# rvolden/C3POa

Measured on AMD Instinct MI355X. Metric: R2C2 reads->consensus/sec, higher is better.
Workload: dtype int32

## Files before the change

### c3poa_amd/csrc/c3_args.h

```cpp
#pragma once
#include "c3_dev.h"
#include <cstddef>

struct C3Counters {
  int queue;
  int peaks_queue;
  unsigned long long cells;
  unsigned long long cells_computed;
  unsigned long long zero_cells;
  int poa_ovf;
  int poa_ovf16;
  int n_windows;
  int win_ovf;
  int win_queue2;
  int band_layers, band_fallback;
  int band_mismatch;
  struct { int window, layer, R, q, band_row, full_row, next_row; } verify;
  unsigned long long phases[16];
};
static_assert(offsetof(C3Counters, cells) % 8 == 0 && offsetof(C3Counters, cells_computed) % 8 == 0 &&
              offsetof(C3Counters, zero_cells) % 8 == 0 && offsetof(C3Counters, phases) % 8 == 0, "u64 counters must be 8-byte aligned");

struct ConkArgs {
  C3Batch b; const uint8_t* sp_codes; const int* sp_len; int32_t* track; C3Info* info; C3Counters* cnt;
  int match, mismatch, penalty;
  int n_spl; int32_t* scan;
};
struct PeaksArgs {
  C3Batch b; const int32_t* track; C3Info* info; double* bufA; double* bufB; int32_t* cand; uint8_t* cstate;
  int32_t* raw_peaks; int32_t* n_raw; const int* sp_len; double coef[64]; int64_t maxL; int window, iters, min_dist;
  C3Counters* cnt;
};
struct PoaArgs {
  C3Batch b; C3Info* info; C3Params p; C3Counters* cnt; const int* work; int n_work;
  int* ibase; int* ebase; char* cellsb; uint8_t* bbase; long long* score;
  int Ncap, K, Pcap, cells_cap;
// ... 24 lines not shown
  C3Batch b; C3Info* info; C3Params p; C3Counters* cnt; const int* work; int n_work;
  const uint8_t* draft; int32_t* tpos; int wcap; uint8_t* eD; int64_t ecap; int* lw_first; int* lw_last; int NLcap, NWcap;
  WinRec* wrec; WLayer* wlay; int* win_base;
  int sub_shift;
  int rows_old;
};
struct WinArgs {
  C3Batch b; C3Params p; C3Counters* cnt; int n_win; const WinRec* wrec_in; WinRec* wrec; const WLayer* wlay; int NLcap;
  const uint8_t* draft;
  uint8_t* base; int* ibase; int* ebase; long long* score;
  int32_t* H; uint16_t* D; uint4* rdesc; int Ncap, K; long long hcap; uint8_t* wout; int wout_cap;
  int Lcap;
  int band_mode;
  const int* wlist; int* ovf_list;
  int no_chain;
};
#define W_INTS 19
struct WinLayout { size_t ints, edges, bases, score, H, D, desc, total; };
__host__ __device__ inline WinLayout c3_win_layout(size_t Ncap, size_t K, size_t hcap) {
  WinLayout l;
  l.ints = sizeof(int) * W_INTS * Ncap; l.edges = sizeof(int) * 4 * Ncap * K; l.bases = 2 * Ncap; l.score = sizeof(long long) * Ncap;
  l.H = sizeof(int32_t) * hcap; l.D = hcap; l.desc = sizeof(uint4) * (Ncap + 1);
  l.total = l.ints + l.edges + l.bases + l.score + l.H + l.D + l.desc;
  return l;
}
struct StitchArgs {
  C3Batch b; C3Info* info; const int* work; int n_work; const WinRec* wrec; const int* win_base; const uint8_t* wout; int wout_cap; char* cons;
  const uint8_t* zflag;
};
struct AdapterArgs {
// ... 33 lines not shown
```

### c3poa_amd/csrc/c3_handle.hip

```cpp
#include "c3_host.h"
#include "c3_bgzf.h"

thread_local double c3h::g_alloc_ms = 0.0;

__device__ __forceinline__ uint32_t pack_code(uint32_t b) {
  const uint32_t u = b & 0xDFu;
  const uint32_t c = (u >> 1) & 3u;
  const bool ok = (u == 'A') | (u == 'C') | (u == 'G') | (u == 'T') | (u == 'U');
  return ok ? (c ^ (c >> 1)) : 0u;
}
__global__ __launch_bounds__(256) void k_pack(const uint8_t* ascii, const int64_t* off, const int64_t* woff, int n, uint32_t* pk) {
  const int lane = threadIdx.x & 63;
  const int wave = (blockIdx.x * blockDim.x + threadIdx.x) >> 6, n_waves = (gridDim.x * blockDim.x) >> 6;
  for (int r = wave; r < n; r += n_waves) {
    const int64_t L = off[r + 1] - off[r];
    const int64_t nw = woff[r + 1] - woff[r];
    const uint8_t* s = ascii + off[r];
    uint32_t* dst = pk + woff[r];
    for (int64_t w = lane; w < nw; w += 64) {
      uint32_t x = 0;
      if (w * 16 + 16 <= L) {
        uint32_t v[4];
        __builtin_memcpy(v, s + w * 16, 16);
#pragma unroll
// ... 456 lines not shown
extern "C" int c3_debug_calibrate(c3_handle* h, long long bytes) {
  if (!h || bytes < 4096) return C3_E_ARG;
  HIPCHK(hipSetDevice(h->cfg.device));
  uint32_t *a = nullptr, *b = nullptr;
  HIPCHK(hipMalloc(&a, (size_t)bytes)); HIPCHK(hipMalloc(&b, (size_t)bytes));
  HIPCHK(hipMemsetAsync(a, 1, (size_t)bytes, h->stream));
  HIPCHK(hipStreamSynchronize(h->stream));
  hipLaunchKernelGGL(k_calib_rw, dim3(h->n_cus * 8), dim3(256), 0, h->stream, a, b, (size_t)bytes / 4);
  HIPCHK(hipStreamSynchronize(h->stream));
  HIPCHK(hipFree(a)); HIPCHK(hipFree(b));
  return C3_E_OK;
}

extern "C" int c3_debug_phases(c3_handle* h, int which, unsigned long long* out) {
  if (!h || !out) return C3_E_ARG;
  memcpy(out, which ? h->phase_win : h->phase_poa, 128);
  return C3_E_OK;
}

extern "C" int c3_batch_timing(c3_handle* h, c3_timing* t) { if (!h || !t) return C3_E_ARG; *t = h->tm; return C3_E_OK; }

extern "C" int c3_fetch_track(c3_handle* h, int read, int32_t* out, int64_t cap) {
  if (!h || read < 0 || read >= h->n || !out) return C3_E_ARG;
  if (!(h->stages_done & C3_STAGE_CONK)) return c3_fail(h, C3_E_STATE, "conk stage not run");
  int64_t L = h->off[read + 1] - h->off[read];
  if (cap < L) return C3_E_LIMIT;
  HIPCHK(hipSetDevice(h->cfg.device));
  HIPCHK(hipMemcpy(out, h->d_track.as<int32_t>() + h->off[read], sizeof(int32_t) * (size_t)L, hipMemcpyDeviceToHost));
  return (int)L;
}
extern "C" int c3_fetch_smoothed(c3_handle* h, int read, double* out, int64_t cap) {
// ... 60 lines not shown
```

### c3poa_amd/csrc/c3_host.h

```cpp
#pragma once
#include "c3_dev.h"
#include "c3_args.h"
#include "c3_launch.h"
#include "c3_checks.h"
#include "c3_emit.h"
#include "c3_post.h"
#include "c3_fastx.h"
#include "c3_dsplit.h"
#include "c3_bgzf.h"
#include <algorithm>
#include <atomic>
#include <chrono>
#include <cstddef>
#include <cstdio>
#include <cstdlib>
#include <cstring>
#include <functional>
#include <string>
#include <vector>

struct c3_handle;
namespace c3h {
extern thread_local double g_alloc_ms;
int qv_scratch(c3_handle* h, long long max_m, long long max_n, int n_items, QvArgs& a, int* grid);
// ... 119 lines not shown
  DBuf d_qv, s_qv_dirs, s_qv_g, d_qv_cnt, d_gather_qv;
  hipEvent_t ev_qv[2] = {nullptr, nullptr}; c3_qv_timing qtm = {}; bool snap_qv = false;
  DBuf d_post[16]; hipEvent_t ev_post[5] = {}; c3_post_timing ptm = {};
  PostText pt;
  DemuxText dx; std::vector<uint32_t> dmx_meta_host;
  DBuf d_fa[20]; hipEvent_t ev_fa[10] = {}; c3_demux_timing dtm = {}; struct C3FaHdr* h_fa_hdr = nullptr;
  DBuf d_emit[10]; c3h::EmitBufs emit_sa; c3_emit_timing etm = {};
  c3h::EmitBufs emit_snap; DBuf d_emit_names, d_emit_noff; c3h::ZStage emit_zs;
  hipEvent_t ev_emit_dn = nullptr;
  std::atomic<bool> emit_pending{false}; int emit_S = 0, emit_flags = 0; std::vector<int64_t> emit_so; c3_emit_timing emit_tm = {};
  std::vector<Summary> sum; std::vector<int> work;
  int res_prefix = 0;
  int peaks_grid = 0; bool debug_msa = false; bool injected = false;
  int n_windows = 0;
  c3_timing tm;
  unsigned long long phase_poa[16] = {0}, phase_win[16] = {0};
  int stages_done = 0;
};

static inline int c3_hip_fail(c3_handle* h, hipError_t e, const char* what, const char* file, int line) {
  char buf[512];
  const char* base = strrchr(file, '/');
  snprintf(buf, sizeof buf, "HIP error %d (%s) at %s:%d: %s", (int)e, hipGetErrorString(e), base ? base + 1 : file, line, what);
  if (h) h->err = buf;
  return C3_E_HIP;
}
static inline int c3_fail(c3_handle* h, int code, const char* msg) { if (h) h->err = msg; return code; }
#define HIPCHK(x) do { hipError_t e_ = (x); if (e_ != hipSuccess) return c3_hip_fail(h, e_, #x, __FILE__, __LINE__); } while (0)
static inline int host_fail(int code, const char* msg) { c3_set_host_error(msg); return code; }
static inline int bgzf_fail(hipError_t e, const char* what) {
  char buf[256];
// ... 57 lines not shown
```

### c3poa_amd/csrc/c3_stages.hip

```cpp
#include "c3_host.h"

__global__ void k_summary(const C3Info* info, const int64_t* off, int n, Summary* out) {
  int i = blockIdx.x * blockDim.x + threadIdx.x;
  if (i >= n) return;
  const C3Info* p = &info[i];
  Summary s; s.status = p->status; s.n_sub = p->n_sub; s.max_sub = 0; s.sum_sub = 0; s.max_dang = 0; s.n_peaks = p->n_peaks;
  for (int k = 0; k < p->n_sub; ++k) { int l = p->sub_end[k] - p->sub_beg[k]; s.sum_sub += l; if (l > s.max_sub) s.max_sub = l; }
  int L = (int)(off[i + 1] - off[i]);
  s.front = p->has_front ? p->front_end : 0; s.tail = p->has_tail ? L - p->tail_beg : 0;
  if (p->has_front) s.max_dang = p->front_end;
  if (p->has_tail && L - p->tail_beg > s.max_dang) s.max_dang = L - p->tail_beg;
  out[i] = s;
}

static hipError_t zero_counters(c3_handle* h) { return hipMemsetAsync(h->d_counter.p, 0, sizeof(C3Counters), h->stream); }

static int auto_slots(c3_handle* h, int want, size_t per_slot_bytes, int n_items, int waves_per_cu) {
  int s = want > 0 ? want : h->n_cus * waves_per_cu;
  size_t budget = h->mem_total ? h->mem_total / 3 : ((size_t)64 << 30);
  if (per_slot_bytes > 0) { size_t mx = budget / per_slot_bytes; if ((size_t)s > mx) s = (int)std::max<size_t>(mx, 1); }
  if (s > n_items) s = std::max(n_items, 1);
  return s;
}

// ... 304 lines not shown
      HIPCHK(h->s_win_h2.ensure(L2.H * S2)); HIPCHK(h->s_win_d2.ensure(L2.D * S2 + 256));
      HIPCHK(h->d_wovf.ensure(sizeof(int) * (size_t)n_win));
    }
    WinArgs a; memset(&a, 0, sizeof(a));
    a.b = dev_batch(h); a.p = dev_params(h->cfg); a.cnt = dev_cnt(h); a.n_win = n_win;
    a.wrec_in = h->d_wrec.as<WinRec>(); a.wrec = h->d_wrec.as<WinRec>(); a.wlay = h->d_wlay.as<WLayer>(); a.NLcap = NLcap;
    a.draft = h->d_draft.as<uint8_t>();
    a.ibase = h->s_win_i.as<int>(); a.ebase = h->s_win_nk.as<int>();
    a.base = h->s_win_b.as<uint8_t>(); a.score = h->s_win_sc.as<long long>();
    a.H = h->s_win_h.as<int32_t>(); a.D = h->s_win_d.as<uint16_t>(); a.rdesc = h->s_win_desc.as<uint4>(); a.Ncap = Ncap; a.K = K; a.hcap = hcap; a.Lcap = std::min(std::min(Ncap, 2 * WL + 30 * NLcap), ((getenv("C3_DEBUG_WIN_LDS") ? atoi(getenv("C3_DEBUG_WIN_LDS")) : 6656) - 16) / 6);
    if (const char* e = getenv("C3_DEBUG_WIN_LCAP")) a.Lcap = std::max(64, std::min(Ncap, atoi(e)));
    a.wout = h->d_wout.as<uint8_t>(); a.wout_cap = wout_cap;
    HIPCHK(zero_counters(h));
    if (const char* e = getenv("C3_DEBUG_BAND")) a.band_mode = !strcmp(e, "off") ? 1 : !strcmp(e, "fail") ? 2 : !strcmp(e, "verify") ? 3 : 0;
    if (const char* e = getenv("C3_DEBUG_WIN_CHAIN")) a.no_chain = !strcmp(e, "0");
    a.ovf_list = slots2 ? h->d_wovf.as<int>() : nullptr;
    c3k_launch_window(&a, slots, h->stream);
    HIPCHK(hipGetLastError());
    if (slots2) {
      a.H = h->s_win_h2.as<int32_t>(); a.D = h->s_win_d2.as<uint16_t>(); a.hcap = hcap_full;
      a.wlist = h->d_wovf.as<int>(); a.ovf_list = nullptr;
      c3k_launch_window(&a, slots2, h->stream);
      HIPCHK(hipGetLastError());
    }
    HIPCHK(hipMemcpyAsync(h->phase_win, dev_cnt(h)->phases, sizeof(h->phase_win), hipMemcpyDeviceToHost, h->stream));
  }
  HIPCHK(hipEventRecord(h->ev[8], h->stream));
  StitchArgs s; memset(&s, 0, sizeof(s));
  s.b = dev_batch(h); s.info = h->d_info.as<C3Info>(); s.work = h->d_work.as<int>(); s.n_work = nw;
  s.wrec = h->d_wrec.as<WinRec>(); s.win_base = h->d_wbase.as<int>(); s.wout = h->d_wout.as<uint8_t>(); s.wout_cap = wout_cap;
  s.cons = h->d_cons.as<char>(); s.zflag = h->d_zflag.as<uint8_t>();
  DBG("stitch\n");
  c3k_launch_stitch(&s, std::min(nw, h->n_cus * 16), h->stream);
  HIPCHK(hipGetLastError());
  HIPCHK(hipEventRecord(h->ev[9], h->stream));
  HIPCHK(read_counters(h, &c));
  if (n_win > 0) {
    h->tm.n_win_redo = c.win_ovf; h->tm.cells_polish += c.cells; h->tm.cells_polish_computed += c.cells_computed;
    h->tm.n_band_layers = c.band_layers; h->tm.n_band_fallback = c.band_fallback; h->tm.n_band_mismatch = c.band_mismatch;
    if (c.band_mismatch) fprintf(stderr, "c3poa: band verify mismatch in window %d layer %d (R = %d): last differing base q = %d, band row %d, full row %d, row of q+1 = %d\n",
                                 c.verify.window, c.verify.layer, c.verify.R, c.verify.q, c.verify.band_row, c.verify.full_row, c.verify.next_row);
  }
  HIPCHK(hipEventElapsedTime(ms_prep, h->ev[5], h->ev[6]));
  HIPCHK(hipEventElapsedTime(ms_win, h->ev[7], h->ev[8]));
  HIPCHK(hipEventElapsedTime(ms_st, h->ev[8], h->ev[9]));
  h->tm.n_windows = n_win;
  return 0;
}

static const long long QV_BUDGET = 1LL << 30;
int c3h::qv_scratch(c3_handle* h, long long max_m, long long max_n, int n_items, QvArgs& a, int* grid) {
  a.dir_words = (max_m + 7) / 8 * 64;
  a.lds_n = (int)std::min<long long>((max_n + 15) / 16 * 16, c3k_qv_lds_max());
  a.gcap = max_n > a.lds_n ? (max_n + 15) / 16 * 16 : 0;
// ... 96 lines not shown
```

### c3poa_amd/csrc/k_polish.hip

```cpp
#include "c3_dev.h"
#include "c3_args.h"
#include "c3_launch.h"
#include <algorithm>
#include <type_traits>

#define WSYNC() __syncthreads()
#define EI(v, k) ((size_t)(k) * (size_t)c.Ncap + (size_t)(v))
#ifndef C3_WIN_RING
#define C3_WIN_RING 1
#endif



#ifndef C3_PREP_WAVES
#define C3_PREP_WAVES 5
#endif
#define EC 5
#define EXT_DCAP 4096
#define EXT_STATIC (-(1 << 27))
#define EXT_ECW 8
__device__ inline long long ext_dir_bytes(long long n, int rpw) { return (n / rpw + 1) * 256; }
template <bool DL>
__device__ long long extend_align(const PrepArgs& a, const uint32_t* pk, const uint8_t* draft, const uint8_t* ldraft, int C,
                                  int pb, int n, int dir_, int32_t* tpos, uint8_t* D, int lane) {
// ... 838 lines not shown
  WSYNC();
  return nn;
}

__host__ __device__ __forceinline__ int win_mask_words(int Ncap) { return ((Ncap + 64) >> 6) + 1; }
__host__ __device__ __forceinline__ size_t win_lds_bytes(int Lcap, int Ncap) {
  const size_t masks = (size_t)32 * win_mask_words(Ncap);
  const size_t a = (size_t)Lcap * 6 + 16, b = masks + 4 * 5 * 64 * 4 + 64, c = masks + 4 * (size_t)wb_lds_dwords(639, 4), d = masks + 4 * (size_t)(W_TBW + W_QCAP);
  size_t m = a > b ? a : b; m = m > c ? m : c; m = m > d ? m : d;
  return m;
}

__device__ __forceinline__ int win_idx(int j, int cpl) { return cpl ? (j / cpl) * ((cpl + 3) & ~3) + j % cpl : j; }

__device__ int win_rows_dispatch(WCtx& c, const C3Params& P, const uint32_t* pk, int qbeg, int Q, int R, int lane, int* cpl_out, int* rs_out, unsigned long long* dbg,
                                 unsigned long long* m2, unsigned long long* ma, unsigned long long* d0, unsigned long long* d1, int ring_off, int lds_ints, int begin, int end, int blen, int* cb_io, int* nblocks, const uint8_t* chain_bb, int chain_v0, int MW) {
  const int need = (Q + 1 + 63) / 64;
  int cpl;
  const int pm = max(max(abs(P.pol_match), abs(P.pol_mismatch)), abs(P.pol_gap));
  const bool ok16 = !(4 * pm * (max(R, Q) + 4) >= 31000 || 4 * (abs(P.pol_match) + abs(P.pol_gap)) * (Q + 4) >= 31000 || pm > 30 || P.pol_gap >= 0);
  if (!ok16) cpl = 0;
#ifdef C3_EXP_NOWIDE
  else if (need <= 2) cpl = 2; else if (need <= 4) cpl = 4; else cpl = 0;
#else
  else if (need <= 2) cpl = 2; else if (need <= 4) cpl = 4; else if (need <= 6) cpl = 6; else if (need <= 8) cpl = 8;
  else if (need <= 10) cpl = 10; else cpl = 0;
#endif
  const int span = end - begin + 1;
  int cb = R * 4 < span * 5 ? 2 : R * 2 < span * 3 ? 3 : 4;
  cb = max(cb, *cb_io);
  if (cb > 4) cb = 0;
  if (!*cb_io || !cb || !ok16 || need > 10 || need <= cb || span < 1 || max(P.pol_match, P.pol_mismatch) <= 0 || ring_off + wb_lds_dwords(Q, cb) > lds_ints) cb = 0;
#ifdef C3_BAND_OFF
  cb = 0;
#endif
#ifdef C3_PHASE_PROF
  const unsigned long long bd_t0 = __builtin_readcyclecounter();
#endif
  if (cb && chain_bb) { *nblocks = R; if (!win_chain_desc_band(c.rdesc, chain_bb, chain_v0, R, Q, begin, end, cb, MW)) cb = 0; }
  else if (cb && !win_build_desc_band(c, R, Q, begin, end, blen, cb, lane, m2, ma, d0, d1, nblocks)) cb = 0;
#ifdef C3_EXP_X2_DESC
  if (cb && !win_build_desc_band(c, R, Q, begin, end, blen, cb, lane, m2, ma, d0, d1, nblocks)) cb = 0;
#endif
#ifdef C3_PHASE_PROF
  dbg[5] += __builtin_readcyclecounter() - bd_t0;
#endif
  *cb_io = cb;
  if (cb) {
    *cpl_out = cb; *rs_out = 256;
    int rc = 0;
#ifdef C3_EXP_X2_ROWS
    for (int rep_ = 0; rep_ < 2; ++rep_)
#endif
    switch (cb) {
      case 2: rc = win_rows_band<2>(c.I, c.E, c.H, c.D, c.rdesc, c.K, c.n, c.Ncap, c.hcap, P.pol_match, P.pol_mismatch, P.pol_gap, pk, qbeg, Q, R, dbg, ring_off, *nblocks); break;
      case 3: rc = win_rows_band<3>(c.I, c.E, c.H, c.D, c.rdesc, c.K, c.n, c.Ncap, c.hcap, P.pol_match, P.pol_mismatch, P.pol_gap, pk, qbeg, Q, R, dbg, ring_off, *nblocks); break;
      default: rc = win_rows_band<4>(c.I, c.E, c.H, c.D, c.rdesc, c.K, c.n, c.Ncap, c.hcap, P.pol_match, P.pol_mismatch, P.pol_gap, pk, qbeg, Q, R, dbg, ring_off, *nblocks); break;
// ... 149 lines not shown
  const int slot = blockIdx.x;
  WCtx c;
  const size_t N = (size_t)a.Ncap;
  c.I = a.ibase + (size_t)slot * W_INTS * N; c.E = a.ebase + (size_t)slot * 4 * N * a.K;
  c.B8 = a.base + (size_t)slot * 2 * N; c.score = a.score + slot * N;
  c.H = a.H + (size_t)slot * a.hcap; c.D = (uint8_t*)a.D + (size_t)slot * a.hcap; c.rdesc = a.rdesc + slot * (N + 1);
  c.K = a.K; c.Ncap = a.Ncap; c.hcap = a.hcap;
  const C3Params& P = a.p;
  extern __shared__ int lds_dyn[];
  int* s_score = lds_dyn; unsigned short* s_pred = (unsigned short*)(lds_dyn + a.Lcap);
  const int MW = win_mask_words(a.Ncap);
  unsigned long long* m2bits = (unsigned long long*)lds_dyn; unsigned long long* mabits = m2bits + MW;
  unsigned long long* d0bits = mabits + MW; unsigned long long* d1bits = d0bits + MW;
  const int lds_ints = (int)(win_lds_bytes(a.Lcap, a.Ncap) / 4);
  PH_DECL

  for (;;) {
    int wi = 0;
    if (lane == 0) {
      if (SECOND) {
        wi = atomicAdd(&a.cnt->win_queue2, 1);
        wi = wi < *(const volatile int*)&a.cnt->win_ovf ? a.wlist[wi] : -1;
      } else {
        wi = atomicAdd(&a.cnt->queue, 1);
        if (wi >= a.n_win) wi = -1;
      }
    }
    wi = wave_first(wi);
    if (wi < 0) break;
    PH_MARK(9)
// ... 113 lines not shown
          }
        }
#ifdef C3_EXP_X2_COMP
        WSYNC(); }
#endif
        WSYNC();
        PH_MARK(2)
        const int ring_off = 8 * MW;
        const QArr rq = {(unsigned short*)((unsigned*)lds_dyn + ring_off + W_TBW), c.opq(), Q > W_QCAP};
        const QArr tq = {(unsigned short*)((unsigned*)lds_dyn + ring_off + W_TBW) + W_QCAP, c.opn(), Q > W_QCAP};
        unsigned long long tbp_[4] = {0, 0, 0, 0};
        bool verify = false;
        for (int vpass = 0; vpass < 2 && !fail; ++vpass) {
        int cpl = 0, RS = 0, cb = a.band_mode != 1 && vpass == 0, gbs = INT32_MIN, gbr = 0;
        for (int attempt = 0; attempt < 4; ++attempt) {
          unsigned long long dbg_[6] = {0, 0, 0, 0, 0, 0};
          int nblocks = 0;
          if (win_rows_dispatch(c, P, pk, l.qbeg, Q, R, lane, &cpl, &RS, dbg_, m2bits, mabits, d0bits, d1bits, ring_off, lds_ints, l.begin, l.end, blen, &cb, &nblocks, chain ? bb : nullptr, chain_v0, MW) < 0) { fail = SECOND ? 1 : 2; break; }
#ifdef C3_PHASE_PROF
          ph_acc_[10] += dbg_[0]; ph_acc_[11] += dbg_[1];
#endif
          PH_MARK(3)
          cells_done += (long long)(R + 1) * (cb ? 64 * cb : Q + 1);
          if (cb) {
            WSYNC();
            const int bound = c.lob()[0];
            gbs = c.lob()[1]; gbr = c.lob()[2];
#ifdef C3_EXP_NOCERT
            if (cb) { ++n_band; break; }
#endif
            if (gbs != INT32_MIN && bound < gbs && a.band_mode != 2) { ++n_band; break; }
          } else {
            int bs = INT32_MIN, br = INT32_MAX / 2;
            for (int r = 1 + lane; r <= R; r += 64) { const int sc = c.hend()[r]; if (sc > bs) { bs = sc; br = r; } }
            gbs = wave_max(bs);
// ... 227 lines not shown
      }
    }
    if (fail == 2 && a.ovf_list) {
      if (lane == 0) a.ovf_list[atomicAdd(&a.cnt->win_ovf, 1)] = wi;
    } else if (lane == 0) {
      WinRec* r = &a.wrec[wi];
      r->out_len = fail ? -1 : olen; r->polished = polished;
      atomicAdd(&a.cnt->cells, (unsigned long long)cells);
      atomicAdd(&a.cnt->cells_computed, (unsigned long long)cells_done);
      if (n_band) atomicAdd(&a.cnt->band_layers, n_band);
      if (n_fallback) atomicAdd(&a.cnt->band_fallback, n_fallback);
    }
    WSYNC();
  }
  PH_FLUSH(a.cnt->phases)
}


__global__ __launch_bounds__(64) void k_stitch(StitchArgs a) {
  const int lane = wave_lane();
  for (int wi = blockIdx.x; wi < a.n_work; wi += gridDim.x) {
    const int rid = a.work[wi];
    C3Info* info = &a.info[rid];
    if (info->status != C3_ST_OK) continue;
    if (a.zflag && a.zflag[rid]) continue;
    const int64_t off = a.b.off[rid];
    const int L = (int)(a.b.off[rid + 1] - off);
    const int nwin = info->n_win, wb = a.win_base[rid];
    char* cons = a.cons + off;
    int olen = 0, any = 0, bad = 0;
// ... 24 lines not shown
```

### c3poa_amd/csrc/k_polish_band.h

```cpp
#pragma once

#define WB_PADL 4
#define WB_PADR 28
#define WB_MAXSHIFT 24
#ifndef WB_RING
#define WB_RING 4
#endif
#define WB_EROW 12
#define WB_EROWS 32
__host__ __device__ __forceinline__ int wb_slot_shorts(int cb) { return WB_PADL + 64 * cb + WB_PADR; }
__host__ __device__ __forceinline__ int wb_lds_dwords(int Q, int cb) { return ((Q + 2) & ~1) + WB_RING * wb_slot_shorts(cb) / 2 + WB_EROWS * WB_EROW / 2; }
__device__ __forceinline__ int wb_left(int cb) { return cb == 2 ? 70 : cb == 3 ? 105 : 140; }
__host__ __device__ __forceinline__ int wb_rpw(int cb) { return cb == 2 ? 8 : 4; }
__host__ __device__ __forceinline__ int wb_bit0(int cb) { return 32 - 2 * cb * wb_rpw(cb); }

__device__ __forceinline__ int wb_words(int R, int cb) { return (R + wb_rpw(cb) - 1) / wb_rpw(cb); }

#define WB_W_LO(w) ((int)((w) & 0x3ffu))
#define WB_W_DIST(w) ((int)(((w) >> 10) & 0xffu))
#define WB_W_BIDX(w) ((int)((w) >> 18))
__device__ int win_build_desc_band(WCtx& c, int R, int Q, int begin, int end, int blen, int CB, int lane,
                                   unsigned long long* m2, unsigned long long* ma, unsigned long long* d0, unsigned long long* d1, int* nblocks) {
  const int BW = 64 * CB, WLf = wb_left(CB), span = end - begin + 1, lomax = Q + 1 - BW;
  if (R >= 16000 || Q > 1000) return 0;
  int bbc = begin - 1, loc = 0, nbc = 0, gprev = -1, bad = 0;
#ifndef WB_DU
#define WB_DU 1
#endif
  constexpr int DU = WB_DU;
  for (int rb = 1; rb <= R; rb += 64 * DU) {
    int v[DU], nin[DU], nout[DU], gr[DU], pe[DU][4], se[DU][4];
    unsigned vb[DU];
#pragma unroll
    for (int u = 0; u < DU; ++u) { const int r = rb + 64 * u + lane; v[u] = r <= R ? c.rows()[r] : -1; }
#pragma unroll
    for (int u = 0; u < DU; ++u) {
      const bool live = v[u] >= 0;
      nin[u] = live ? c.n_in()[v[u]] : 0; nout[u] = live ? c.n_out()[v[u]] : 0;
      vb[u] = live ? (unsigned)c.base()[v[u]] & 3u : 0u; gr[u] = live ? c.grp()[v[u]] : -2;
    }
// ... 53 lines not shown
        for (int k = 4; k < nout[u]; ++k) {
          const int sr = c.rowof()[c.out_to()[EI(v[u], k)]];
          if (sr >= 0) { has = 1; dist = max(dist, sr - r); if (sr == r + 1) next = 1; else other = 1; }
        }
        far = dist > WB_RING;
        if (dist > 64) bad = 1;
        ovf = np > 4; virt = np == 0;
        if (np == 0) np = 1;
        two = np == 1;
        adj = two && (int)p[0] == r - 1;
        fast = adj && !far && has && dl <= 1;
#ifdef C3_EXP_NOFAST
        fast = 0;
#endif
      }
      const unsigned fastn = (unsigned)__builtin_amdgcn_update_dpp(0, (int)fast, 0x130, 0xf, 0xf, false);
      if (live) {
        const unsigned wr = other | (next & (fastn ^ 1u));
        uint4 d; d.x = vb[u] * 8u | ((unsigned)min(np, 255) << 8) | (ovf << 16) | (far << 17) | ((has ^ 1u) << 18) | ((unsigned)two << 19) | (fast << 20)
                       | ((unsigned)(fast ? dl : 0) << 22) | (wr << 23) | (virt << 24);
        d.y = p[0] | (p[1] << 16); d.z = p[2] | (p[3] << 16); d.w = (unsigned)lo | ((unsigned)min(dist, 255) << 10) | ((unsigned)bidx << 18);
        c.rdesc[r] = d;
      }
      const unsigned long long b2 = __ballot(two), ba = __ballot(adj), bd0 = __ballot(dl & 1), bd1 = __ballot((dl & 2) != 0);
      if (lane == 0) { m2[r0 >> 6] = b2; ma[r0 >> 6] = ba; d0[r0 >> 6] = bd0; d1[r0 >> 6] = bd1; }
    }
  }
  *nblocks = nbc;
  bad = __ballot(bad) != 0;
  WSYNC();
  return !bad;
}

__device__ __attribute__((noinline)) int win_chain_desc_band(uint4* crdesc, const uint8_t* bb_, int v0_, int R_, int Q_, int begin_, int end_, int CB_, int mw_) {
  uint4* const rdesc = uni_ptr(crdesc);
  const uint8_t* const bb = uni_ptr(bb_);
  const int v0 = uni32(v0_), R = uni32(R_), Q = uni32(Q_), begin = uni32(begin_), end = uni32(end_), CB = uni32(CB_), MW = uni32(mw_);
// ... 96 lines not shown
  int cV = g4 + 2;
  VREG(cV);
  WSYNC();
  const unsigned* tp = tbl + CB * lane;
  int lo = 0;
  unsigned tn[CB + 1];
#pragma unroll
  for (int k = 0; k <= CB; ++k) tn[k] = tp[k];
  unsigned dacc = 0;
  unsigned dwoff = (unsigned)lane;
  const unsigned ebase = (unsigned)(size_t)(__attribute__((address_space(3))) unsigned short*)ebuf + 2u * (lane < 2 ? (unsigned)(lane * CB) : 8u);
  int best = (BW - 1) * gap + ups * (Q - BW + 1);
  int ebs = INT32_MIN, ebr = INT32_MAX / 2, bandbad = 0;
#ifdef C3_PHASE_PROF
  unsigned long long pf_fast = 0, pf_d0 = 0, pf_d1 = 0, pf_c2 = 0, pf_c3 = 0, pf_c4 = 0;
#endif

#define WB_ROW_TAIL(PIDX)                                                                                        \
    {                                                                                                            \
      int run = W_NEG16;                                                                                         \
      _Pragma("unroll") for (int cc = 0; cc < CB; ++cc) run = max16(run, key[cc] - g41[cc]);                    \
      int ex = wave_shr1(wave_scan_max(__builtin_amdgcn_sbfe(run, 0, 16)), W_NEG16);                             \
      unsigned w2 = 0, pidx = 0;                                                                                 \
      _Pragma("unroll") for (int cc = 0; cc < CB; ++cc) {                                                       \
        const int k2 = max16(key[cc], (ex & ~3) + g41[cc]);                                                      \
        ex = max16(ex, key[cc] - g41[cc]);                                                                       \
        hcur[cc] = k2 & ~3;                                                                                      \
        w2 |= ((unsigned)k2 & 3u) << (32 - BPR + 2 * cc);                                                        \
        if (PIDX) pidx |= (((unsigned)key[cc] >> 16) & 63u) << (8 * cc);                                         \
      }                                                                                                          \
      dacc = (dacc >> BPR) | w2;                                                                                 \
      if (PIDX) GP(unsigned, PX)[(unsigned)r * 64u + (unsigned)lane] = pidx;                                     \
      wb_park_edge<CB>(ebase + (unsigned)(li & (WB_EROWS - 1)) * (2u * WB_EROW), hcur);                                             \
    }
#define WB_RING_WRITE()                                                                                          \
    {                                                                                                            \
      unsigned short* sp_ = ring + (r & (WB_RING - 1)) * SLOT;                                                   \
      *(int*)sp_ = lo;                                                                                           \
      _Pragma("unroll") for (int cc = 0; cc < CB; ++cc) sp_[WB_PADL + CB * lane + cc] = (unsigned short)hcur[cc]; \
    }

  for (int rb = 1; rb <= R; rb += 64) {
    typedef unsigned u32x4 __attribute__((ext_vector_type(4)));
    const u32x4 dv = GP(const u32x4, c.rdesc)[min(rb + lane, R)];
    uint4 dblk = make_uint4(dv.x, dv.y, dv.z, dv.w);
    asm volatile("" : "+v"(dblk.x), "+v"(dblk.y), "+v"(dblk.z), "+v"(dblk.w));
    const int cnt = min(64, R - rb + 1);
    for (int half_ = 0; half_ < 64 && half_ < cnt; half_ += WB_EROWS) {
    const int hend_ = min(half_ + WB_EROWS, cnt);
    for (int li = half_; li < hend_; ++li) {
      const int r = rb + li;
      const unsigned dx = (unsigned)__builtin_amdgcn_readlane((int)dblk.x, li);
      int key[CB];
      if (dx & (1u << 20)) {
        const int vb8 = (int)(dx & 24u);
#ifdef C3_PHASE_PROF
        ++pf_fast;
#endif
        if (dx & (1u << 22)) {
          int tv[CB];
#pragma unroll
          for (int cc = 0; cc < CB; ++cc) tv[cc] = __builtin_amdgcn_sbfe((int)tn[cc + 1], vb8, 8);
          lo += 1;
#pragma unroll
          for (int k = 0; k <= CB; ++k) tn[k] = tp[lo + k];
          const int hnext = wave_shl1(hcur[0], W_NEG16);
#pragma unroll
          for (int cc = 0; cc < CB; ++cc) {
// ... 2 lines not shown
          }
          WB_ROW_TAIL(false)
        } else {
          int tv[CB];
#pragma unroll
          for (int cc = 0; cc < CB; ++cc) tv[cc] = __builtin_amdgcn_sbfe((int)tn[cc], vb8, 8);
          const int hleft = wave_shr1(hcur[CB - 1], W_NEG16);
#pragma unroll
          for (int cc = 0; cc < CB; ++cc) {
            const int hd = cc == 0 ? hleft : hcur[cc > 0 ? cc - 1 : 0];
            key[cc] = max16(hd + tv[cc], hcur[cc] + cV);
          }
          WB_ROW_TAIL(false)
        }
        if (dx & (1u << 23)) WB_RING_WRITE()
      } else {
#ifdef C3_PHASE_PROF
        const unsigned long long gen_t0 = __builtin_readcyclecounter();
#endif
        uint4 de;
        de.x = dx;
        de.y = __builtin_amdgcn_readlane(dblk.y, li);
        de.z = __builtin_amdgcn_readlane(dblk.z, li);
        de.w = __builtin_amdgcn_readlane(dblk.w, li);
        const int np = (de.x >> 8) & 0xff;
        const bool ovf = (de.x >> 16) & 1, two = (de.x >> 19) & 1;
        if (np > 64) return -1;
        lo = WB_W_LO(de.w);
        const int vb8 = (int)(dx & 24u);
        int tv[CB];
#pragma unroll
        for (int cc = 0; cc < CB; ++cc) tv[cc] = __builtin_amdgcn_sbfe((int)tp[lo + cc], vb8, 8);
#pragma unroll
// ... 43 lines not shown
        }
        if (two) WB_ROW_TAIL(false) else WB_ROW_TAIL(true)
        if (de.x & (1u << 23)) WB_RING_WRITE()
        if ((de.x >> 17) & 1) {
          auto* hrow = GP(unsigned short, H16) + (size_t)r * HS;
          hrow[0] = (unsigned short)lo; hrow[1] = (unsigned short)((unsigned)lo >> 16);
#pragma unroll
          for (int cc = 0; cc < CB; ++cc) hrow[WB_PADL + CB * lane + cc] = (unsigned short)hcur[cc];
        }
        if ((de.x >> 18) & 1) {
#pragma unroll
          for (int cc = 0; cc < CB; ++cc) { const int sc = __builtin_amdgcn_sbfe(hcur[cc], 2, 14); if (lo + lane * CB + cc == Q && sc > ebs) { ebs = sc; ebr = r; } }
        }
#ifdef C3_PHASE_PROF
        { const bool pm1 = (de.y & 0xffff) == (unsigned)(r - 1); pf_d0 += (1ull << 32) + (two && pm1); pf_d1 += 1 + ((unsigned long long)!two << 32);
          const unsigned long long dt_ = __builtin_readcyclecounter() - gen_t0; if (!two) pf_c2 += dt_; else if (pm1) pf_c4 += dt_; else pf_c3 += dt_; }
#endif
      }
      if ((li & (RPW - 1)) == RPW - 1) { GP(unsigned, DW)[dwoff] = dacc; dwoff += 64; dacc = 0; }
    }
    if (hend_ == cnt && (cnt & (RPW - 1))) {
      const int miss = RPW - (cnt & (RPW - 1));
      GP(unsigned, DW)[dwoff] = dacc >> (BPR * miss); dwoff += 64; dacc = 0;
    }
    if (lane >= half_ && lane < hend_) {
      const unsigned short* e = ebuf + (lane & (WB_EROWS - 1)) * WB_EROW;
      const int r = rb + lane;
      const int lo_r = WB_W_LO(dblk.w), dist = WB_W_DIST(dblk.w), nb = NB - WB_W_BIDX(dblk.w);
      const int hi = lo_r + BW - 1;
      if (hi < Q) best = max(best, ((int)(short)e[8 + CB - 1] >> 2) + ups * (Q - hi));
      if (((dblk.x >> 24) & 1) && lo_r > 0) best = max(best, ups * min(Q, nb + 1) + gap * max(0, Q - nb - 1));
// ... 2 lines not shown
        unsigned long long a0 = d0bits[w0] >> off, a1 = d1bits[w0] >> off;
        if (off) { a0 |= d0bits[w0 + 1] << (64 - off); a1 |= d1bits[w0 + 1] << (64 - off); }
        const unsigned long long dm = dist >= 64 ? ~0ull : ((1ull << dist) - 1ull);
        const int ls = __popcll(a0 & dm) + 2 * __popcll(a1 & dm);
        if (ls > 2 * CB) bandbad = 1;
        for (int b = 0; b < min(ls, 2 * CB); ++b) {
          const int rem = Q - lo_r - b;
          best = max(best, ((int)(short)e[b] >> 2) + ups * min(rem, nb) + gap * max(0, rem - nb));
        }
      }
    }
    }
  }
#undef WB_ROW_TAIL
#undef WB_RING_WRITE
  best = wave_max(best);
  const int gbs = wave_max(ebs);
  const int gbr = wave_min(ebs == gbs ? ebr : INT32_MAX / 2);
  if (lane == 0) { auto* res = GP(int, c.lob().ptr()); res[0] = best; res[1] = gbs; res[2] = gbr; }
  bandbad = __ballot(bandbad) != 0;
#ifdef C3_PHASE_PROF
  dbg[0] += pf_d0; dbg[1] += pf_d1 + pf_fast; dbg[2] += pf_c2; dbg[3] += pf_c3; dbg[4] += pf_c4;
#endif
  WSYNC();
  return bandbad ? 1 : 0;
}

#ifndef WB_TB_SHIFT
#define WB_TB_SHIFT 3
#endif
__device__ __attribute__((noinline)) void win_traceback_band(int* cI, int* cE, uint8_t* cD, uint4* crdesc, int cK, int cn, int cNcap, int CB_, int R_, int Q_, int r_,
                                                             int mw_, int big_, unsigned long long* prof_) {
  WCtx c;
  c.I = uni_ptr(cI); c.E = uni_ptr(cE); c.B8 = nullptr; c.score = nullptr; c.H = nullptr; c.D = uni_ptr(cD);
  c.rdesc = uni_ptr(crdesc); c.K = uni32(cK); c.n = uni32(cn); c.Ncap = uni32(cNcap); c.hcap = 0;
  const int CB = uni32(CB_), R = uni32(R_), Q = uni32(Q_), MW = uni32(mw_);
  int r = uni32(r_);
// ... 134 lines not shown
```

Measured before the change: 427,600.

## Add ring-buffer fast path for banded window rows with near predecessors

Adds a third row path to the banded window DP. Rows with one or two predecessors within the last WB_RING rows and a small band shift read predecessor scores directly from the LDS ring, using offsets precomputed into the descriptor. This avoids the general predecessor-gather path for these rows. The descriptor builder gains extra cross-lane permute and broadcast work per row, and debug counters and an env knob to disable or count the path are added.

Result: no change. 430,200, median of 4 (+0.6%).

```diff
diff --git a/c3poa_amd/csrc/c3_args.h b/c3poa_amd/csrc/c3_args.h
--- a/c3poa_amd/csrc/c3_args.h
+++ b/c3poa_amd/csrc/c3_args.h
@@ -16,10 +16,11 @@
   int band_layers, band_fallback;
   int band_mismatch;
   struct { int window, layer, R, q, band_row, full_row, next_row; } verify;
-  unsigned long long phases[16];
+  unsigned long long phases[32];
+  unsigned long long ring_rows[16];
 };
 static_assert(offsetof(C3Counters, cells) % 8 == 0 && offsetof(C3Counters, cells_computed) % 8 == 0 &&
-              offsetof(C3Counters, zero_cells) % 8 == 0 && offsetof(C3Counters, phases) % 8 == 0, "u64 counters must be 8-byte aligned");
+              offsetof(C3Counters, zero_cells) % 8 == 0 && offsetof(C3Counters, phases) % 8 == 0 && offsetof(C3Counters, ring_rows) % 8 == 0, "u64 counters must be 8-byte aligned");
 
 struct ConkArgs {
   C3Batch b; const uint8_t* sp_codes; const int* sp_len; int32_t* track; C3Info* info; C3Counters* cnt;
@@ -74,6 +75,7 @@
   int band_mode;
   const int* wlist; int* ovf_list;
   int no_chain;
+  int ring_mode;
 };
 #define W_INTS 19
 struct WinLayout { size_t ints, edges, bases, score, H, D, desc, total; };
diff --git a/c3poa_amd/csrc/c3_handle.hip b/c3poa_amd/csrc/c3_handle.hip
--- a/c3poa_amd/csrc/c3_handle.hip
+++ b/c3poa_amd/csrc/c3_handle.hip
@@ -494,7 +494,13 @@
 
 extern "C" int c3_debug_phases(c3_handle* h, int which, unsigned long long* out) {
   if (!h || !out) return C3_E_ARG;
-  memcpy(out, which ? h->phase_win : h->phase_poa, 128);
+  memcpy(out, which == 2 ? h->phase_win + 16 : which ? h->phase_win : h->phase_poa, 128);
+  return C3_E_OK;
+}
+
+extern "C" int c3_debug_ring_rows(c3_handle* h, unsigned long long* out) {
+  if (!h || !out) return C3_E_ARG;
+  memcpy(out, h->ring_rows, sizeof(h->ring_rows));
   return C3_E_OK;
 }
 
diff --git a/c3poa_amd/csrc/c3_host.h b/c3poa_amd/csrc/c3_host.h
--- a/c3poa_amd/csrc/c3_host.h
+++ b/c3poa_amd/csrc/c3_host.h
@@ -157,7 +157,8 @@
   int peaks_grid = 0; bool debug_msa = false; bool injected = false;
   int n_windows = 0;
   c3_timing tm;
-  unsigned long long phase_poa[16] = {0}, phase_win[16] = {0};
+  unsigned long long phase_poa[16] = {0}, phase_win[32] = {0};
+  unsigned long long ring_rows[16] = {0};
   int stages_done = 0;
 };
 
diff --git a/c3poa_amd/csrc/c3_stages.hip b/c3poa_amd/csrc/c3_stages.hip
--- a/c3poa_amd/csrc/c3_stages.hip
+++ b/c3poa_amd/csrc/c3_stages.hip
@@ -342,6 +342,7 @@
     HIPCHK(zero_counters(h));
     if (const char* e = getenv("C3_DEBUG_BAND")) a.band_mode = !strcmp(e, "off") ? 1 : !strcmp(e, "fail") ? 2 : !strcmp(e, "verify") ? 3 : 0;
     if (const char* e = getenv("C3_DEBUG_WIN_CHAIN")) a.no_chain = !strcmp(e, "0");
+    if (const char* e = getenv("C3_DEBUG_WIN_RING")) a.ring_mode = !strcmp(e, "0") ? 1 : !strcmp(e, "count") ? 2 : 0;
     a.ovf_list = slots2 ? h->d_wovf.as<int>() : nullptr;
     c3k_launch_window(&a, slots, h->stream);
     HIPCHK(hipGetLastError());
@@ -366,6 +367,7 @@
   if (n_win > 0) {
     h->tm.n_win_redo = c.win_ovf; h->tm.cells_polish += c.cells; h->tm.cells_polish_computed += c.cells_computed;
     h->tm.n_band_layers = c.band_layers; h->tm.n_band_fallback = c.band_fallback; h->tm.n_band_mismatch = c.band_mismatch;
+    memcpy(h->ring_rows, c.ring_rows, sizeof(h->ring_rows));
     if (c.band_mismatch) fprintf(stderr, "c3poa: band verify mismatch in window %d layer %d (R = %d): last differing base q = %d, band row %d, full row %d, row of q+1 = %d\n",
                                  c.verify.window, c.verify.layer, c.verify.R, c.verify.q, c.verify.band_row, c.verify.full_row, c.verify.next_row);
   }
diff --git a/c3poa_amd/csrc/k_polish.hip b/c3poa_amd/csrc/k_polish.hip
--- a/c3poa_amd/csrc/k_polish.hip
+++ b/c3poa_amd/csrc/k_polish.hip
@@ -876,7 +876,8 @@
 __device__ __forceinline__ int win_idx(int j, int cpl) { return cpl ? (j / cpl) * ((cpl + 3) & ~3) + j % cpl : j; }
 
 __device__ int win_rows_dispatch(WCtx& c, const C3Params& P, const uint32_t* pk, int qbeg, int Q, int R, int lane, int* cpl_out, int* rs_out, unsigned long long* dbg,
-                                 unsigned long long* m2, unsigned long long* ma, unsigned long long* d0, unsigned long long* d1, int ring_off, int lds_ints, int begin, int end, int blen, int* cb_io, int* nblocks, const uint8_t* chain_bb, int chain_v0, int MW) {
+                                 unsigned long long* m2, unsigned long long* ma, unsigned long long* d0, unsigned long long* d1, int ring_off, int lds_ints, int begin, int end, int blen, int* cb_io, int* nblocks, const uint8_t* chain_bb, int chain_v0, int MW,
+                                 int ring_mode, unsigned long long* ring_cnt) {
   const int need = (Q + 1 + 63) / 64;
   int cpl;
   const int pm = max(max(abs(P.pol_match), abs(P.pol_mismatch)), abs(P.pol_gap));
@@ -900,9 +901,9 @@
   const unsigned long long bd_t0 = __builtin_readcyclecounter();
 #endif
   if (cb && chain_bb) { *nblocks = R; if (!win_chain_desc_band(c.rdesc, chain_bb, chain_v0, R, Q, begin, end, cb, MW)) cb = 0; }
-  else if (cb && !win_build_desc_band(c, R, Q, begin, end, blen, cb, lane, m2, ma, d0, d1, nblocks)) cb = 0;
+  else if (cb && !win_build_desc_band(c, R, Q, begin, end, blen, cb, lane, m2, ma, d0, d1, nblocks, ring_mode, ring_cnt)) cb = 0;
 #ifdef C3_EXP_X2_DESC
-  if (cb && !win_build_desc_band(c, R, Q, begin, end, blen, cb, lane, m2, ma, d0, d1, nblocks)) cb = 0;
+  if (cb && !win_build_desc_band(c, R, Q, begin, end, blen, cb, lane, m2, ma, d0, d1, nblocks, ring_mode, ring_cnt)) cb = 0;
 #endif
 #ifdef C3_PHASE_PROF
   dbg[5] += __builtin_readcyclecounter() - bd_t0;
@@ -1082,6 +1083,9 @@
   unsigned long long* d0bits = mabits + MW; unsigned long long* d1bits = d0bits + MW;
   const int lds_ints = (int)(win_lds_bytes(a.Lcap, a.Ncap) / 4);
   PH_DECL
+#ifdef C3_PHASE_PROF
+  unsigned long long ph_rows_[16] = {0, 0, 0, 0, 0, 0, 0, 0, 0, 0, 0, 0, 0, 0, 0, 0};
+#endif
 
   for (;;) {
     int wi = 0;
@@ -1225,11 +1229,17 @@
         for (int vpass = 0; vpass < 2 && !fail; ++vpass) {
         int cpl = 0, RS = 0, cb = a.band_mode != 1 && vpass == 0, gbs = INT32_MIN, gbr = 0;
         for (int attempt = 0; attempt < 4; ++attempt) {
+#ifdef C3_PHASE_PROF
+          unsigned long long dbg_[22] = {0, 0, 0, 0, 0, 0, 0, 0, 0, 0, 0, 0, 0, 0, 0, 0, 0, 0, 0, 0, 0, 0};
+#else
           unsigned long long dbg_[6] = {0, 0, 0, 0, 0, 0};
+#endif
           int nblocks = 0;
-          if (win_rows_dispatch(c, P, pk, l.qbeg, Q, R, lane, &cpl, &RS, dbg_, m2bits, mabits, d0bits, d1bits, ring_off, lds_ints, l.begin, l.end, blen, &cb, &nblocks, chain ? bb : nullptr, chain_v0, MW) < 0) { fail = SECOND ? 1 : 2; break; }
+          if (win_rows_dispatch(c, P, pk, l.qbeg, Q, R, lane, &cpl, &RS, dbg_, m2bits, mabits, d0bits, d1bits, ring_off, lds_ints, l.begin, l.end, blen, &cb, &nblocks, chain ? bb : nullptr, chain_v0, MW,
+                                a.ring_mode, a.cnt->ring_rows) < 0) { fail = SECOND ? 1 : 2; break; }
 #ifdef C3_PHASE_PROF
           ph_acc_[10] += dbg_[0]; ph_acc_[11] += dbg_[1];
+          for (int i_ = 0; i_ < 16; ++i_) ph_rows_[i_] += dbg_[6 + i_];
 #endif
           PH_MARK(3)
           cells_done += (long long)(R + 1) * (cb ? 64 * cb : Q + 1);
@@ -1487,6 +1497,9 @@
     WSYNC();
   }
   PH_FLUSH(a.cnt->phases)
+#ifdef C3_PHASE_PROF
+  if (lane == 0) { for (int i_ = 0; i_ < 16; ++i_) atomicAdd(a.cnt->phases + 16 + i_, ph_rows_[i_]); }
+#endif
 }
 
 
diff --git a/c3poa_amd/csrc/k_polish_band.h b/c3poa_amd/csrc/k_polish_band.h
--- a/c3poa_amd/csrc/k_polish_band.h
+++ b/c3poa_amd/csrc/k_polish_band.h
@@ -20,10 +20,13 @@
 #define WB_W_DIST(w) ((int)(((w) >> 10) & 0xffu))
 #define WB_W_BIDX(w) ((int)((w) >> 18))
 __device__ int win_build_desc_band(WCtx& c, int R, int Q, int begin, int end, int blen, int CB, int lane,
-                                   unsigned long long* m2, unsigned long long* ma, unsigned long long* d0, unsigned long long* d1, int* nblocks) {
+                                   unsigned long long* m2, unsigned long long* ma, unsigned long long* d0, unsigned long long* d1, int* nblocks,
+                                   int ring_mode, unsigned long long* ring_cnt) {
   const int BW = 64 * CB, WLf = wb_left(CB), span = end - begin + 1, lomax = Q + 1 - BW;
   if (R >= 16000 || Q > 1000) return 0;
   int bbc = begin - 1, loc = 0, nbc = 0, gprev = -1, bad = 0;
+  static_assert(WB_RING <= 4, "the carry below holds the band starts of four rows");
+  int lc1 = 0, lc2 = 0, lc3 = 0, lc4 = 0;
 #ifndef WB_DU
 #define WB_DU 1
 #endif
@@ -107,13 +110,38 @@
         fast = 0;
 #endif
       }
+      unsigned ringrow = live && ring_mode != 1 && !fast && !virt && !ovf && !far && has && np <= 2, zoff = 0;
+#pragma unroll
+      for (int k = 0; k < 2; ++k) {
+        const int pd = k < np ? r - (int)p[k] : 1;
+        const int src = lane - pd;
+        const int plo = __builtin_amdgcn_ds_bpermute((src & 63) << 2, lo);
+        const int sh = lo - (src >= 0 ? plo : src == -1 ? lc1 : src == -2 ? lc2 : src == -3 ? lc3 : lc4);
+        if (pd < 1 || pd > WB_RING || sh < 0 || sh > WB_MAXSHIFT) ringrow = 0;
+        if (k < np) zoff |= ((p[k] & (unsigned)(WB_RING - 1)) * (unsigned)wb_slot_shorts(CB) + (unsigned)(WB_PADL - 1 + sh)) << (16 * k);
+      }
+      lc1 = wave_bcast(lo, 63); lc2 = wave_bcast(lo, 62); lc3 = wave_bcast(lo, 61); lc4 = wave_bcast(lo, 60);
       const unsigned fastn = (unsigned)__builtin_amdgcn_update_dpp(0, (int)fast, 0x130, 0xf, 0xf, false);
       if (live) {
         const unsigned wr = other | (next & (fastn ^ 1u));
         uint4 d; d.x = vb[u] * 8u | ((unsigned)min(np, 255) << 8) | (ovf << 16) | (far << 17) | ((has ^ 1u) << 18) | ((unsigned)two << 19) | (fast << 20)
-                       | ((unsigned)(fast ? dl : 0) << 22) | (wr << 23) | (virt << 24);
-        d.y = p[0] | (p[1] << 16); d.z = p[2] | (p[3] << 16); d.w = (unsigned)lo | ((unsigned)min(dist, 255) << 10) | ((unsigned)bidx << 18);
+                       | (ringrow << 21) | ((unsigned)(fast ? dl : 0) << 22) | (wr << 23) | (virt << 24) | ((unsigned)(ringrow ? dl : 0) << 25);
+        d.y = p[0] | (p[1] << 16); d.z = ringrow ? zoff : p[2] | (p[3] << 16); d.w = (unsigned)lo | ((unsigned)min(dist, 255) << 10) | ((unsigned)bidx << 18);
         c.rdesc[r] = d;
+      }
+      if (ring_mode == 2) {
+        const int rpw = wb_rpw(CB), pd0 = r - (int)p[0], pd1 = np == 2 ? r - (int)p[1] : 0;
+        const unsigned rr = ringrow, abv = (unsigned)wave_shr1z((int)(ringrow | ((unsigned)(fast && dl == 1) << 1)));
+        const unsigned shp = rr | (rr & (unsigned)(np == 1)) << 1 | (rr & (unsigned)(np == 2)) << 2 | (rr & (unsigned)(pd0 == WB_RING || pd1 == WB_RING)) << 3
+            | (unsigned)(live && !rr && !fast && !virt && !ovf && np <= 2 && (pd0 == WB_RING + 1 || pd1 == WB_RING + 1)) << 4
+            | (rr & (unsigned)(lane == 0 && r0 > 1)) << 5 | (rr & (unsigned)(lane == 63)) << 6 | (rr & (unsigned)(r % WB_EROWS == 0)) << 7
+            | (rr & (unsigned)(lane % WB_EROWS == 0)) << 8 | (rr & (unsigned)(R % rpw != 0 && r > R - R % rpw)) << 9
+            | (rr & (unsigned)(np == 2 && p[0] > p[1])) << 10 | (rr & abv & 1u) << 11 | (rr & (abv >> 1) & 1u) << 12;
+#pragma nounroll
+        for (int i = 0; i < 13; ++i) {
+          const int cn = __popcll(__ballot((shp >> i) & 1u));
+          if (lane == 0 && cn) atomicAdd(ring_cnt + i, (unsigned long long)cn);
+        }
       }
       const unsigned long long b2 = __ballot(two), ba = __ballot(adj), bd0 = __ballot(dl & 1), bd1 = __ballot((dl & 2) != 0);
       if (lane == 0) { m2[r0 >> 6] = b2; ma[r0 >> 6] = ba; d0[r0 >> 6] = bd0; d1[r0 >> 6] = bd1; }
@@ -240,6 +268,7 @@
   int ebs = INT32_MIN, ebr = INT32_MAX / 2, bandbad = 0;
 #ifdef C3_PHASE_PROF
   unsigned long long pf_fast = 0, pf_d0 = 0, pf_d1 = 0, pf_c2 = 0, pf_c3 = 0, pf_c4 = 0;
+  unsigned long long pf_cf = 0, pf_cr1 = 0, pf_cr2 = 0, pf_nr1 = 0, pf_nr2 = 0, pf_g2 = 0, pf_gnear = 0, pf_gplain = 0, pf_gall = 0, pf_n2 = 0, pf_n3 = 0, pf_n4 = 0;
 #endif
 
 #define WB_ROW_TAIL(PIDX)                                                                                        \
@@ -266,6 +295,25 @@
       _Pragma("unroll") for (int cc = 0; cc < CB; ++cc) sp_[WB_PADL + CB * lane + cc] = (unsigned short)hcur[cc]; \
     }
 
+#define WB_RING_ROW(NP)                                                                                          \
+    {                                                                                                            \
+      int hp[NP][CB + 1];                                                                                        \
+      _Pragma("unroll") for (int t = NP - 1; t >= 0; --t) {                                                     \
+        const unsigned short* cp = ring + CB * lane + ((dz >> (16 * t)) & 0xffffu);                              \
+        _Pragma("unroll") for (int k = 0; k <= CB; ++k) hp[t][k] = (int)cp[k];                                   \
+      }                                                                                                          \
+      _Pragma("unroll") for (int k = 0; k <= CB; ++k) tn[k] = tp[lo + k];                                       \
+      _Pragma("unroll") for (int cc = 0; cc < CB; ++cc) {                                                       \
+        const int tv = __builtin_amdgcn_sbfe((int)tn[cc], vb8, 8);                                               \
+        key[cc] = max16(hp[0][cc] + tv, hp[0][cc + 1] + cV);                                                     \
+        if (NP == 2) {                                                                                           \
+          const int nk = max16(key[cc], max16(hp[NP - 1][cc] + tv, hp[NP - 1][cc + 1] + cV));                    \
+          key[cc] = nk != (key[cc] & 0xffff) ? (nk | (1 << 16)) : key[cc];                                       \
+        }                                                                                                        \
+      }                                                                                                          \
+      WB_ROW_TAIL(NP == 2)                                                                                       \
+    }
+
   for (int rb = 1; rb <= R; rb += 64) {
     typedef unsigned u32x4 __attribute__((ext_vector_type(4)));
     const u32x4 dv = GP(const u32x4, c.rdesc)[min(rb + lane, R)];
@@ -278,6 +326,9 @@
       const int r = rb + li;
       const unsigned dx = (unsigned)__builtin_amdgcn_readlane((int)dblk.x, li);
       int key[CB];
+#ifdef C3_PHASE_PROF
+      const unsigned long long row_t0 = __builtin_readcyclecounter();
+#endif
       if (dx & (1u << 20)) {
         const int vb8 = (int)(dx & 24u);
 #ifdef C3_PHASE_PROF
@@ -310,9 +361,21 @@
           WB_ROW_TAIL(false)
         }
         if (dx & (1u << 23)) WB_RING_WRITE()
+#ifdef C3_PHASE_PROF
+        pf_cf += __builtin_readcyclecounter() - row_t0;
+#endif
+      } else if (dx & (1u << 21)) {
+        const unsigned dz = (unsigned)__builtin_amdgcn_readlane((int)dblk.z, li);
+        const int vb8 = (int)(dx & 24u);
+        lo += (int)((dx >> 25) & 3u);
+        if (dx & (1u << 19)) WB_RING_ROW(1) else WB_RING_ROW(2)
+        if (dx & (1u << 23)) WB_RING_WRITE()
+#ifdef C3_PHASE_PROF
+        { const unsigned long long dt_ = __builtin_readcyclecounter() - row_t0; if (dx & (1u << 19)) { pf_cr1 += dt_; ++pf_nr1; } else { pf_cr2 += dt_; ++pf_nr2; } }
+#endif
       } else {
 #ifdef C3_PHASE_PROF
-        const unsigned long long gen_t0 = __builtin_readcyclecounter();
+        const unsigned long long gen_t0 = row_t0;
 #endif
         uint4 de;
         de.x = dx;
@@ -386,7 +449,11 @@
         }
 #ifdef C3_PHASE_PROF
         { const bool pm1 = (de.y & 0xffff) == (unsigned)(r - 1); pf_d0 += (1ull << 32) + (two && pm1); pf_d1 += 1 + ((unsigned long long)!two << 32);
-          const unsigned long long dt_ = __builtin_readcyclecounter() - gen_t0; if (!two) pf_c2 += dt_; else if (pm1) pf_c4 += dt_; else pf_c3 += dt_; }
+          const unsigned long long dt_ = __builtin_readcyclecounter() - gen_t0; if (!two) { pf_c2 += dt_; ++pf_n2; } else if (pm1) { pf_c4 += dt_; ++pf_n4; } else { pf_c3 += dt_; ++pf_n3; }
+          const bool virt_ = (de.x >> 24) & 1, plain_ = !virt_ && !ovf && !((de.x >> 17) & 3);
+          bool near_ = !virt_ && !ovf;
+          for (int t = 0; t < np && t < 4 && near_; ++t) near_ = r - (int)((t < 2 ? de.y : de.z) >> (16 * (t & 1)) & 0xffff) <= WB_RING;
+          pf_g2 += np <= 2; pf_gnear += near_; pf_gplain += plain_; pf_gall += np <= 2 && near_ && plain_; }
 #endif
       }
       if ((li & (RPW - 1)) == RPW - 1) { GP(unsigned, DW)[dwoff] = dacc; dwoff += 64; dacc = 0; }
@@ -419,6 +486,7 @@
   }
 #undef WB_ROW_TAIL
 #undef WB_RING_WRITE
+#undef WB_RING_ROW
   best = wave_max(best);
   const int gbs = wave_max(ebs);
   const int gbr = wave_min(ebs == gbs ? ebr : INT32_MAX / 2);
@@ -426,6 +494,8 @@
   bandbad = __ballot(bandbad) != 0;
 #ifdef C3_PHASE_PROF
   dbg[0] += pf_d0; dbg[1] += pf_d1 + pf_fast; dbg[2] += pf_c2; dbg[3] += pf_c3; dbg[4] += pf_c4;
+  dbg[6] += pf_c2; dbg[7] += pf_c3; dbg[8] += pf_c4; dbg[9] += pf_cf; dbg[10] += pf_fast; dbg[11] += pf_cr1; dbg[12] += pf_cr2; dbg[13] += pf_nr1; dbg[14] += pf_nr2;
+  dbg[15] += pf_g2; dbg[16] += pf_gnear; dbg[17] += pf_gplain; dbg[18] += pf_gall; dbg[19] += pf_n2; dbg[20] += pf_n3; dbg[21] += pf_n4;
 #endif
   WSYNC();
   return bandbad ? 1 : 0;
```
